# svohr/mixemt

Measured on AMD Instinct MI355X. Metric: read x hap cells/sec through the EM iteration (EM iters/sec reported beside it as em_iters_per_s), 1000000 reads x 5408 haps in total, whole job, higher is better.
Workload: dtype f64

## Files before the change

### mixemt_amd/csrc/coded_kernels.hpp

```cpp
#ifndef MIXEMT_CODED_KERNELS_HPP
#define MIXEMT_CODED_KERNELS_HPP

#define ENC_THREADS 256
#define ENC_SLOTS 1024
#define ENC_MAX_CODES 256
#define ENC_MAX_WIDE 1024
#define ENC_WIDE_SLOTS 4096
#define ENC_EMPTY 0xFFFFFFFFFFFFFFFFull

__host__ __device__ __forceinline__ int rec_code_bytes(int nd, int ldc) { return nd > ENC_MAX_CODES ? 2 * ldc : ldc; }
__device__ __forceinline__ int rec_code_at(const uint8_t *codes, int h, bool wide) {
    return wide ? (int)reinterpret_cast<const uint16_t *>(codes)[h] : (int)codes[h];
}

template <int NCH, bool WIDE>
__device__ __forceinline__ void encode_one_row(int64_t r, const double *__restrict__ M, int64_t ldm, int H, int ldc,
                                               uint8_t *__restrict__ rec, int64_t rec_cap, int64_t *__restrict__ rec_off,
                                               int32_t *__restrict__ ndist, double *__restrict__ rowmax,
                                               unsigned long long *__restrict__ stats) {
    constexpr int NW = ENC_THREADS / 64;
    constexpr int SLOTS = WIDE ? ENC_WIDE_SLOTS : ENC_SLOTS;
    constexpr int MAXC = WIDE ? ENC_MAX_WIDE : ENC_MAX_CODES;
    constexpr int SPT = SLOTS / ENC_THREADS;
    __shared__ unsigned long long s_key[SLOTS];
    __shared__ unsigned short s_code[SLOTS];
    __shared__ double s_red[NW];
    __shared__ int s_wcnt[NW];
    __shared__ int s_flag, s_n;
    __shared__ long long s_off;
    const int t = threadIdx.x, lane = t & 63, wv = t >> 6;
    typedef unsigned int u4 __attribute__((ext_vector_type(4)));
    typedef unsigned int u2 __attribute__((ext_vector_type(2)));

    const auto rsrc = __builtin_amdgcn_make_buffer_rsrc(const_cast<double *>(M + r * ldm), 0, H * 8, 0x00020000);
    double x[NCH][4];
#pragma unroll
    for (int k = 0; k < NCH; ++k) {
        const int off = (t + k * ENC_THREADS) * 32;
        const d2 a = __builtin_bit_cast(d2, (u4)__builtin_amdgcn_raw_buffer_load_b128(rsrc, off, 0, 2));
        const d2 b = __builtin_bit_cast(d2, (u4)__builtin_amdgcn_raw_buffer_load_b128(rsrc, off, 16, 2));
        x[k][0] = a.x;
        x[k][1] = a.y;
        x[k][2] = b.x;
        x[k][3] = b.y;
    }
    if (H & 1) {
        const double tail = M[r * ldm + (H - 1)];
#pragma unroll
        for (int k = 0; k < NCH; ++k) {
            if (4 * (t + k * ENC_THREADS) == H - 1) x[k][0] = tail;
            if (4 * (t + k * ENC_THREADS) + 2 == H - 1) x[k][2] = tail;
        }
    }
#pragma unroll
    for (int q = 0; q < SPT; ++q) s_key[t + q * ENC_THREADS] = ENC_EMPTY;
    if (t == 0) {
        s_flag = 0;
        s_n = 0;
    }
    double m = -INFINITY;
#pragma unroll
    for (int k = 0; k < NCH; ++k)
#pragma unroll
        for (int e = 0; e < 4; ++e)
            if (4 * (t + k * ENC_THREADS) + e < H) m = fmax(m, x[k][e]);
    m = wave_max(m);
    if (lane == 0) s_red[wv] = m;
    __syncthreads();
    m = fmax(fmax(s_red[0], s_red[1]), fmax(s_red[2], s_red[3]));
    const double shift = isfinite(m) ? m : 0.0;

    int slot[NCH][4];
    unsigned long long prev_key = ENC_EMPTY;
    int prev_slot = 0;
#pragma unroll
    for (int k = 0; k < NCH; ++k) {
        const bool give_up = *(volatile int *)&s_flag != 0;
#pragma unroll
        for (int e = 0; e < 4; ++e) {
            const bool valid = 4 * (t + k * ENC_THREADS) + e < H;
            const unsigned long long key = (unsigned long long)__double_as_longlong(x[k][e]);
            int sl = 0;
            bool need = valid;
            if (valid && key == ENC_EMPTY) {
                s_flag = 1;
                need = false;
            }
            if (need && key == prev_key) {
                sl = prev_slot;
                need = false;
            }
            if (give_up) need = false;
            if (need) {
                unsigned int h = (unsigned int)((key ^ (key >> 29)) * 0x9E3779B97F4A7C15ull >> 40) & (SLOTS - 1);
                for (int probes = 0;; ++probes) {
                    const unsigned long long old = atomicCAS(&s_key[h], ENC_EMPTY, key);
                    if (old == ENC_EMPTY) {
                        if (atomicAdd(&s_n, 1) >= MAXC) s_flag = 1;
                        break;
                    }
                    if (old == key) break;
                    h = (h + 1) & (SLOTS - 1);
                    if (probes >= SLOTS) {
                        s_flag = 1;
                        break;
                    }
                }
                sl = (int)h;
            }
            slot[k][e] = sl;
            if (valid) {
                prev_key = key;
                prev_slot = sl;
            }
        }
    }
    __syncthreads();
    const bool dense = (s_flag != 0);

    int cnt = 0;
#pragma unroll
    for (int j = 0; j < SPT; ++j) cnt += (s_key[SPT * t + j] != ENC_EMPTY) ? 1 : 0;
    const int incl = wave_inclusive_scan_i32(cnt);
    if (lane == 63) s_wcnt[wv] = incl;
    __syncthreads();
    int base = 0, D = 0;
#pragma unroll
    for (int q = 0; q < NW; ++q) {
        if (q < wv) base += s_wcnt[q];
        D += s_wcnt[q];
    }
    const int cbytes = WIDE ? 2 * ldc : ldc;
    const int64_t bytes = (int64_t)cbytes + 16 * (int64_t)D;
    const bool coded = !dense && D <= MAXC && (!WIDE || D > ENC_MAX_CODES);
    if (t == 0) {
        long long off = -1;
        if (coded) {
            off = (long long)atomicAdd(&stats[0], (unsigned long long)bytes);
            if (off + bytes > rec_cap) off = -1;
        }
        s_off = off;
    }
    int code = base + incl - cnt;
#pragma unroll
    for (int j = 0; j < SPT; ++j) {
        if (s_key[SPT * t + j] != ENC_EMPTY) s_code[SPT * t + j] = (unsigned short)code++;
    }
    __syncthreads();
    const long long off = s_off;
    if (off >= 0) {
        double *tbl = reinterpret_cast<double *>(rec + off + cbytes);
        code = base + incl - cnt;
#pragma unroll
        for (int j = 0; j < SPT; ++j) {
            const unsigned long long kk = s_key[SPT * t + j];
            if (kk != ENC_EMPTY) {
                const double mval = __longlong_as_double((long long)kk);
                tbl[code] = exp(mval - shift);
                tbl[D + code] = mval;
                ++code;
            }
        }
#pragma unroll
        for (int k = 0; k < NCH; ++k) {
            const int c0 = 4 * (t + k * ENC_THREADS);
            if (c0 < ldc) {
                unsigned int cd[4];
#pragma unroll
                for (int e = 0; e < 4; ++e) cd[e] = (c0 + e < H) ? (unsigned int)s_code[slot[k][e]] : 0u;
                if constexpr (WIDE) {
                    u2 word;
                    word.x = cd[0] | (cd[1] << 16);
                    word.y = cd[2] | (cd[3] << 16);
                    reinterpret_cast<u2 *>(rec + off)[t + k * ENC_THREADS] = word;
                } else {
                    reinterpret_cast<unsigned int *>(rec + off)[t + k * ENC_THREADS] =
                        cd[0] | (cd[1] << 8) | (cd[2] << 16) | (cd[3] << 24);
                }
            }
        }
    }
    if (t == 0) {
        if constexpr (WIDE) {
            if (off >= 0) {
                ndist[r] = D;
                rec_off[r] = off;
                atomicAdd(&stats[1], ~0ull);
            }
        } else {
            rowmax[r] = shift;
            ndist[r] = (off >= 0) ? D : 0;
            rec_off[r] = (off >= 0) ? off : 0;
            if (off < 0) atomicAdd(&stats[1], 1ull);
        }
    }
    __syncthreads();
}

template <int NCH>
__global__ __launch_bounds__(ENC_THREADS) void encode_rows_kernel(
    const double *__restrict__ M, int64_t ldm, int64_t R, int H, int ldc, uint8_t *__restrict__ rec, int64_t rec_cap,
    int64_t *__restrict__ rec_off, int32_t *__restrict__ ndist, double *__restrict__ rowmax,
    unsigned long long *__restrict__ stats) {
    for (int64_t r = blockIdx.x; r < R; r += gridDim.x)
        encode_one_row<NCH, false>(r, M, ldm, H, ldc, rec, rec_cap, rec_off, ndist, rowmax, stats);
}

template <int NCH>
__global__ __launch_bounds__(ENC_THREADS) void encode_wide_rows_kernel(
    const double *__restrict__ M, int64_t ldm, int64_t R, int H, int ldc, uint8_t *__restrict__ rec, int64_t rec_cap,
    int64_t *__restrict__ rec_off, int32_t *__restrict__ ndist, double *__restrict__ rowmax,
    unsigned long long *__restrict__ stats) {
    constexpr int CH = 32;
    __shared__ int s_list[CH];
    __shared__ int s_nlist;
    const int t = threadIdx.x;
    const int64_t nchunk = (R + CH - 1) / CH;
    for (int64_t c = blockIdx.x; c < nchunk; c += gridDim.x) {
        if (t == 0) s_nlist = 0;
        __syncthreads();
        const int64_t r = c * CH + t;
        if (t < CH && r < R && ndist[r] == 0) s_list[atomicAdd(&s_nlist, 1)] = t;
        __syncthreads();
        const int n = s_nlist;
        for (int i = 0; i < n; ++i)
            encode_one_row<NCH, true>(c * CH + s_list[i], M, ldm, H, ldc, rec, rec_cap, rec_off, ndist, rowmax, stats);
        __syncthreads();
    }
}

template <int THREADS, int NCH, int NBUF, bool NT, bool RESIDENT, bool WIDE_PREFETCH, bool CHECK = false>
__device__ __forceinline__ void coded_row_pass(const uint8_t *__restrict__ rec, const int64_t *__restrict__ rec_off,
                                               const int32_t *__restrict__ ndist, int ldc, const double *__restrict__ w,
                                               const int64_t *__restrict__ wide_rows, int64_t n_wide, int64_t R,
                                               const double (&p)[NCH][4], double (&acc)[NCH][4], bool &meta_ready,
                                               int *chk_result = nullptr, const int64_t *__restrict__ row_list = nullptr,
                                               int64_t n_list = 0, const int32_t *__restrict__ nquad = nullptr, int vbid = -1,
                                               int vgrid = 0) {
    static_assert(NBUF >= 3, "codes NBUF - 1 rows ahead, tables NBUF - 2");
    constexpr int NW = THREADS / 64;
    constexpr int AUX = NT ? 2 : 0;
    __shared__ double s_tbl[NBUF][ENC_MAX_CODES];
    __shared__ __attribute__((aligned(16))) double red[NBUF][NW];
    const int t = threadIdx.x, lane = t & 63, wv = t >> 6;
    const int nword = ldc >> 2;
    const int64_t bid = vbid >= 0 ? (int64_t)vbid : (int64_t)blockIdx.x, grid = vbid >= 0 ? (int64_t)vgrid : (int64_t)gridDim.x;
    const row_deal deal(row_list != nullptr ? n_list : R, bid, grid);
    const int voff = t * 4;
    int last_w = t + (NCH - 1) * THREADS;
    if (last_w > nword - 1) last_w = nword - 1;
    const int voff_last = last_w * 4;
    const bool tbl_thread = (THREADS <= ENC_MAX_CODES) || t < ENC_MAX_CODES;
    const int tslot = t & (ENC_MAX_CODES - 1);
    typedef unsigned int u2v __attribute__((ext_vector_type(2)));
    __shared__ int s_chk[2];
    if constexpr (CHECK) {
        if (t == 0) s_chk[0] = s_chk[1] = 0;
        __syncthreads();
    }
    auto list_row = [&](int64_t e) -> int64_t {
        int64_t r = wide_rows[e];
        if constexpr (CHECK) {
            if (r < 0 || r >= R || (e > 0 && wide_rows[e - 1] >= r)) {
                s_chk[1] = 1;
                r = -1;
            }
        }
        return r;
    };
    auto list_nd = [&](int64_t r) -> int {
        if (r < 0) return 0;
        int nd = ndist[r];
        if constexpr (CHECK) {
            if (nd <= ENC_MAX_CODES) {
                s_chk[1] = 1;
                nd = 0;
            }
        }
        return nd;
    };

    __shared__ long long s_off[2][THREADS];
    __shared__ double s_wr[2][THREADS];
    __shared__ int s_nd[2][THREADS];
    auto fetch_meta = [&](int half, int64_t q0) {
        const int64_t q = q0 + t;
        int64_t r = deal.row(q);
        bool struck = false;
        if (row_list != nullptr) {
            const int64_t e = r;
            r = row_list[e];
            if constexpr (CHECK) {
                if (r < 0 || r >= R || (e > 0 && row_list[e - 1] >= r)) {
                    s_chk[1] = 1;
                    r = 0;
                    struck = true;
                }
            }
        }
        int nd = ndist[r];
        if (nd > ENC_MAX_CODES) {
            if constexpr (CHECK) {
                if (row_list != nullptr) s_chk[1] = 1;
                else if (deal.live(q)) atomicAdd(&s_chk[0], 1);
            }
            nd = 0;
        }
        if constexpr (CHECK) {
            if (row_list != nullptr && !struck && (nd <= 0 || nquad[r] != 0)) {
                s_chk[1] = 1;
                struck = true;
            }
        }
        if (struck) nd = 0;
        s_off[half][t] = rec_off[r];
        s_nd[half][t] = nd;
        s_wr[half][t] = (deal.live(q) && nd > 0) ? (w != nullptr ? w[r] : 1.0) : 0.0;
    };

    unsigned int cw[NBUF][NCH];
    double tring[NBUF];
    int pre_off_lo, pre_off_hi, pre_nd;
    double pre_wr;
    auto read_meta = [&](int64_t q_load, int64_t q_weight) {
        const int half = (int)((q_load / THREADS) & 1), idx = (int)(q_load % THREADS);
        const long long off = s_off[half][idx];
        pre_nd = __builtin_amdgcn_readfirstlane(s_nd[half][idx]);
        pre_off_hi = __builtin_amdgcn_readfirstlane((int)(off >> 32));
        pre_off_lo = __builtin_amdgcn_readfirstlane((int)off);
        pre_wr = s_wr[(q_weight / THREADS) & 1][q_weight % THREADS];
    };
    auto load_row = [&](unsigned int(&cws)[NCH], double &tbl_entry) {
        const int nd = pre_nd;
        const uint8_t *base = rec + (((long long)pre_off_hi << 32) | (unsigned int)pre_off_lo);
        const auto rs = __builtin_amdgcn_make_buffer_rsrc(const_cast<uint8_t *>(base), 0, ldc, 0x00020000);
#pragma unroll
        for (int k = 0; k < NCH - 1; ++k) cws[k] = __builtin_amdgcn_raw_buffer_load_b32(rs, voff, k * THREADS * 4, AUX);
        cws[NCH - 1] = __builtin_amdgcn_raw_buffer_load_b32(rs, voff_last, 0, AUX);
        if (tbl_thread) {
            const auto rt = __builtin_amdgcn_make_buffer_rsrc(const_cast<uint8_t *>(base + ldc), 0, nd * 8, 0x00020000);
            const u2v v = __builtin_amdgcn_raw_buffer_load_b64(rt, tslot * 8, 0, AUX);
            tbl_entry = __hiloint2double((int)v.y, (int)v.x);
        }
    };

    const unsigned int three = 3;
    auto entry_off = [&](unsigned int word, auto E) -> unsigned int {
        constexpr int e = decltype(E)::value;
        unsigned int r;
        if constexpr (e == 0) asm("v_lshlrev_b32_sdwa %0, %1, %2 dst_sel:DWORD dst_unused:UNUSED_PAD src0_sel:DWORD src1_sel:BYTE_0" : "=v"(r) : "v"(three), "v"(word));
        else if constexpr (e == 1) asm("v_lshlrev_b32_sdwa %0, %1, %2 dst_sel:DWORD dst_unused:UNUSED_PAD src0_sel:DWORD src1_sel:BYTE_1" : "=v"(r) : "v"(three), "v"(word));
        else if constexpr (e == 2) asm("v_lshlrev_b32_sdwa %0, %1, %2 dst_sel:DWORD dst_unused:UNUSED_PAD src0_sel:DWORD src1_sel:BYTE_2" : "=v"(r) : "v"(three), "v"(word));
        else asm("v_lshlrev_b32_sdwa %0, %1, %2 dst_sel:DWORD dst_unused:UNUSED_PAD src0_sel:DWORD src1_sel:BYTE_3" : "=v"(r) : "v"(three), "v"(word));
        return r;
    };
    auto lookup = [&](const char *tb, unsigned int word, auto E) -> double {
        return *reinterpret_cast<const double *>(tb + entry_off(word, E));
    };
    using E0 = std::integral_constant<int, 0>;
    using E1 = std::integral_constant<int, 1>;
    using E2 = std::integral_constant<int, 2>;
    using E3 = std::integral_constant<int, 3>;

    double v[NCH][4];
    auto lookup_row = [&](const char *tb, const unsigned int(&cws)[NCH]) {
#pragma unroll
        for (int k = 0; k < NCH; ++k) {
            v[k][0] = lookup(tb, cws[k], E0{});
            v[k][1] = lookup(tb, cws[k], E1{});
            v[k][2] = lookup(tb, cws[k], E2{});
            v[k][3] = lookup(tb, cws[k], E3{});
        }
    };

    auto step = [&](auto J, int64_t q) {
        constexpr int j = decltype(J)::value;
        constexpr int jn = (j + 1) % NBUF, jl = (j + NBUF - 1) % NBUF;
        if constexpr (!RESIDENT) {
            if ((q % THREADS) == 0) fetch_meta((int)((q / THREADS + 1) & 1), q + THREADS);
        }
// ... 343 lines not shown
```

### mixemt_amd/csrc/mixemt_hip.hip

```cpp
#include <hip/hip_runtime.h>
#include <stdint.h>
#include <stdio.h>
#include <stdlib.h>
#include <string.h>
#include <math.h>
#include <algorithm>
#include <atomic>
#include <mutex>
#include <type_traits>
#include <utility>
#include <vector>

#include "mixemt_hip.h"
#include "mixemt_hip_tuning.h"

#include "common.hpp"
#include "aln_encode.hpp"
#include "bam_reader.hpp"
#include "coded_kernels.hpp"
#include "quad_kernels.hpp"
#include "quad_batched_kernels.hpp"
#include "build_kernels.hpp"
#include "build_lut_kernels.hpp"
#include "build_sparse_kernels.hpp"
// ... 633 lines not shown
static int em_iter_f32_one(const float *P, int64_t ldp, const double *w, const double *props, int64_t R, int H,
                           const mxm_em_state *state, double *colsum, double *partial, hipStream_t stream,
                           bool timed) {
    const int64_t ldpart = part_ld(H);
    const int nch = ((H + 3) / 4 + MXM_F32_THREADS - 1) / MXM_F32_THREADS;
    const int nbuf = MXM_F32_NBUF;
    int cap = num_cu() * MXM_F32_WG_PER_CU;
    if (cap > MXM_MAX_WG) cap = MXM_MAX_WG;
    const int nwg = clamp_grid((R + nbuf - 1) / nbuf, cap);
    if (timed && T.ev_start != nullptr) HIP_TRY(hipEventRecord(T.ev_start, stream));
    switch (nch) {
#define F32_CASE(n) case n: { const int lrc = launch_wide_f32<n>(P, ldp, w, props, R, H, nwg, partial, ldpart, state, stream); if (lrc != 0) return lrc; } break;
        F32_CASE(1) F32_CASE(2) F32_CASE(3) F32_CASE(4) F32_CASE(5) F32_CASE(6) F32_CASE(7) F32_CASE(8)
#undef F32_CASE
        default: return fail(-1, "mxm_em_iter_f32: H=%s%lld outside the kernel's range", "", H);
    }
    HIP_TRY(hipGetLastError());
    if (timed && T.ev_stop != nullptr) HIP_TRY(hipEventRecord(T.ev_stop, stream));
    hipLaunchKernelGGL(colreduce_kernel, dim3((H + 63) / 64, 1), dim3(COLRED_THREADS), 0, stream, partial, ldpart, nwg,
                       1, H, (const double *)nullptr, colsum, const_cast<mxm_em_state *>(state), slots_from(0), wide_check{nullptr, 0, 0});
    HIP_TRY(hipGetLastError());
    return 0;
}

#define MXM_NARROW_MAX_H 64
template <bool ITER>
static int launch_narrow(const double *M, int64_t ldm, const double *w, const double *ln_props, int64_t R, int H,
                         double *out, int64_t ldo, int mode, double *partial, int64_t ldpart,
                         const mxm_em_state *state, hipStream_t stream, int *nwg_out) {
    const int cap = num_cu() * 4 < MXM_MAX_WG ? num_cu() * 4 : MXM_MAX_WG;
    const int rows_per_wg = (H <= 32) ? 256 : 128;
    const int nwg = clamp_grid((R + rows_per_wg - 1) / rows_per_wg, cap);
    *nwg_out = nwg;
#define NARROW_LAUNCH(hmax, lpr)                                                                             \
    hipLaunchKernelGGL((estep_narrow_kernel<hmax, ITER, lpr>), dim3(nwg), dim3(256), 0, stream, M, ldm, w, ln_props, R, H, \
                       out, ldo, mode, partial, ldpart, state)
    if (H <= 4) NARROW_LAUNCH(4, 1);
    else if (H <= 8) NARROW_LAUNCH(8, 1);
    else if (H <= 16) NARROW_LAUNCH(16, 1);
    else if (H <= 32) NARROW_LAUNCH(32, 1);
    else NARROW_LAUNCH(32, 2);
#undef NARROW_LAUNCH
    HIP_TRY(hipGetLastError());
    return 0;
}

static int em_iter_log_one(const double *M, int64_t ldm, const double *w, const double *ln_props, int64_t R, int H,
                           const mxm_em_state *state, double *colsum, double *partial, hipStream_t stream) {
    if (M == nullptr) return fail(-1, "mxm_em_iter: M is NULL and the linear path does not apply%s", "");
    if (ln_props == nullptr) return fail(-1, "mxm_em_iter: ln_props is NULL and the log-space path needs it%s", "");
    const size_t lds = 2 * (size_t)H * sizeof(double);
    const int64_t ldpart = part_ld(H);
    int nwg;
    if (lds > 150 * 1024) {
        nwg = clamp_grid(R, num_cu() * 2 < MXM_MAX_WG ? num_cu() * 2 : MXM_MAX_WG);
        hipLaunchKernelGGL((estep_global_kernel<true>), dim3(nwg), dim3(ROW_THREADS), 0, stream, M, ldm, w, ln_props, R, H,
                           (double *)nullptr, (int64_t)0, 0, partial, ldpart, state, (const int64_t *)nullptr);
        HIP_TRY(hipGetLastError());
    } else if (H <= MXM_NARROW_MAX_H) {
        const int rc = launch_narrow<true>(M, ldm, w, ln_props, R, H, (double *)nullptr, (int64_t)0, 0, partial, ldpart,
                                           state, stream, &nwg);
        if (rc != 0) return rc;
    } else {
        nwg = clamp_grid(R, num_cu() * 2 < MXM_MAX_WG ? num_cu() * 2 : MXM_MAX_WG);
        if (lds > 60 * 1024 && raise_dynamic_lds(reinterpret_cast<const void *>(&estep_log_kernel<true>), lds, "estep_log_kernel") != hipSuccess)
            return -2;
        hipLaunchKernelGGL((estep_log_kernel<true>), dim3(nwg), dim3(ROW_THREADS), lds, stream, M, ldm, w, ln_props,
                           R, H, (double *)nullptr, (int64_t)0, 0, partial, ldpart, state);
        HIP_TRY(hipGetLastError());
    }
    hipLaunchKernelGGL(colreduce_kernel, dim3((H + 63) / 64, 1), dim3(COLRED_THREADS), 0, stream, partial, ldpart, nwg, 1,
                       H, (const double *)nullptr, colsum, const_cast<mxm_em_state *>(state), slots_from(0), wide_check{nullptr, 0, 0});
    HIP_TRY(hipGetLastError());
    return 0;
}

extern "C" int mxm_em_iter(const double *M, int64_t ldm, const double *P, int64_t ldp, const double *w,
                           const double *props, const double *ln_props, int64_t R, int32_t H, int32_t B,
                           const mxm_em_state *state, double *colsum, void *ws, size_t ws_bytes, void *stream) {
    MXM_ENTER();
    if (R <= 0 || H <= 0 || B <= 0) return fail(-1, "mxm_em_iter: bad shape R=%s%lld H=%lld", "", R, H);
    if (ws == nullptr || ws_bytes < mxm_workspace_bytes(R, H, B)) return fail(-1, "mxm_em_iter: workspace too small%s", "");
    if (P != nullptr && ((ldp & 1) || ldp < H)) return fail(-1, "mxm_em_iter: ldp must be even and >= H%s", "");
    if (M != nullptr && ldm < H) return fail(-1, "mxm_em_iter: ldm < H%s", "");
    const bool linear = (P != nullptr) && mxm_linear_supported(H);
    int max_bt = linear ? T.max_bt : 1;
    while (max_bt > 1 && !batch_fits((int)H, max_bt)) --max_bt;
    for (int b = 0; b < B;) {
        const int left = B - b;
        const int passes = (left + max_bt - 1) / max_bt;
        const int nb = (left + passes - 1) / passes;
        const mxm_em_state *st = state ? state + b : nullptr;
        int rc;
        if (linear)
            rc = em_iter_linear_tile(P, ldp, w, props, R, (int)H, nb, slots_from(b), state, colsum, (double *)ws,
                                     (hipStream_t)stream, b == 0);
        else
            rc = em_iter_log_one(M, ldm, w, ln_props ? ln_props + (int64_t)b * H : nullptr, R, (int)H, st,
                                 colsum + (int64_t)b * H, (double *)ws, (hipStream_t)stream);
        if (rc != 0) return rc;
        b += nb;
    }
    return 0;
}

extern "C" int mxm_linearize_f32(const double *M, int64_t ldm, int64_t R, int32_t H, float *P, int64_t ldp,
                                 double *rowmax, void *stream) {
    if (R < 0 || H <= 0) return fail(-1, "mxm_linearize_f32: bad shape%s", "");
    if (ldm < H || ldp < H || (ldp & 3)) return fail(-1, "mxm_linearize_f32: ldp must be a multiple of 4 and >= H%s (ldp=%lld)", "", ldp);
    if (R == 0) return 0;
    if (wide_rows_ok(M, ldm, H) && (reinterpret_cast<uintptr_t>(P) & 7) == 0 && (ldp & 1) == 0 &&
        linearize_wide<float>(M, ldm, R, (int)H, P, ldp, rowmax, (hipStream_t)stream) == 0) {
        HIP_TRY(hipGetLastError());
        return 0;
    }
    const int grid = clamp_grid(R, num_cu() * 8);
    hipLaunchKernelGGL(linearize_f32_kernel, dim3(grid), dim3(ROW_THREADS), 0, (hipStream_t)stream, M, ldm, R, (int)H,
                       P, ldp, rowmax);
    HIP_TRY(hipGetLastError());
    return 0;
}

extern "C" int mxm_em_iter_f32(const float *P, int64_t ldp, const double *w, const double *props, int64_t R,
                               int32_t H, int32_t B, const mxm_em_state *state, double *colsum, void *ws,
                               size_t ws_bytes, void *stream) {
    MXM_ENTER();
    if (R <= 0 || H <= 0 || B <= 0) return fail(-1, "mxm_em_iter_f32: bad shape R=%s%lld H=%lld", "", R, H);
    if (!mxm_linear_supported(H)) return fail(-1, "mxm_em_iter_f32: H=%s%lld outside the linear kernel's range", "", H);
    if (P == nullptr || (ldp & 3) || ldp < H) return fail(-1, "mxm_em_iter_f32: ldp must be a multiple of 4 and >= H%s", "");
    if (ws == nullptr || ws_bytes < mxm_workspace_bytes(R, H, B)) return fail(-1, "mxm_em_iter_f32: workspace too small%s", "");
    for (int b = 0; b < B; ++b) {
        const int rc = em_iter_f32_one(P, ldp, w, props + (int64_t)b * H, R, (int)H, state ? state + b : nullptr,
                                       colsum + (int64_t)b * H, (double *)ws, (hipStream_t)stream, b == 0);
        if (rc != 0) return rc;
    }
    return 0;
}

extern "C" size_t mxm_coded_bytes(int64_t R, int32_t H) { return mxm_record_bytes(R, H); }

extern "C" int mxm_encode_rows(const double *M, int64_t ldm, int64_t R, int32_t H, uint8_t *rec, size_t rec_bytes,
                               int64_t *rec_off, int32_t *ndist, double *rowmax, int64_t *stats, void *stream) {
    if (R <= 0 || H <= 0 || ldm < H) return fail(-1, "mxm_encode_rows: bad shape R=%s%lld H=%lld", "", R, H);
    if (!mxm_linear_supported(H) || (reinterpret_cast<uintptr_t>(M) & 7) != 0)
        return fail(-1, "mxm_encode_rows: needs H in [65, 8192]%s (H=%lld ldm=%lld)", "", H, ldm);
    if (rec == nullptr || (reinterpret_cast<uintptr_t>(rec) & 15) || rec_bytes < (size_t)coded_ld(H) + 16 * ENC_MAX_CODES)
        return fail(-1, "mxm_encode_rows: record buffer missing, unaligned or smaller than one record%s", "");
    if (rec_off == nullptr || ndist == nullptr || rowmax == nullptr || stats == nullptr)
        return fail(-1, "mxm_encode_rows: output arrays required%s", "");
    hipStream_t s = (hipStream_t)stream;
    HIP_TRY(hipMemsetAsync(stats, 0, 2 * sizeof(int64_t), s));
    const int ldc = coded_ld(H);
    const int nch = (ldc / 4 + ENC_THREADS - 1) / ENC_THREADS;
    const int grid = clamp_grid(R, num_cu() * 4);
    const int grid_w = clamp_grid((R + 31) / 32, num_cu() * 3);
    switch (nch) {
#define ENC_CASE(n) case n: hipLaunchKernelGGL((encode_rows_kernel<n>), dim3(grid), dim3(ENC_THREADS), 0, s, M, ldm, R, (int)H, ldc, rec, (int64_t)rec_bytes, rec_off, ndist, rowmax, reinterpret_cast<unsigned long long *>(stats)); \
                    hipLaunchKernelGGL((encode_wide_rows_kernel<n>), dim3(grid_w), dim3(ENC_THREADS), 0, s, M, ldm, R, (int)H, ldc, rec, (int64_t)rec_bytes, rec_off, ndist, rowmax, reinterpret_cast<unsigned long long *>(stats)); break;
        ENC_CASE(1) ENC_CASE(2) ENC_CASE(3) ENC_CASE(4) ENC_CASE(5) ENC_CASE(6) ENC_CASE(7) ENC_CASE(8)
#undef ENC_CASE
        default: return fail(-1, "mxm_encode_rows: H=%s%lld outside the kernel's range", "", H);
    }
    HIP_TRY(hipGetLastError());
    return 0;
}

static int coded_check(const mxm_coded *c, int32_t H, const char *who) {
    if (c == nullptr || c->R <= 0 || H <= 0 || !mxm_linear_supported(H))
        return fail(-1, "%s: bad coded matrix (rows %lld, H %lld)", who, c ? c->R : 0, H);
    if (c->rec == nullptr || c->rec_off == nullptr || c->ndist == nullptr) return fail(-1, "%s: coded matrix arrays missing", who);
    if (c->R_rest < 0 || (c->R_rest > 0 && (c->P_rest == nullptr || c->ldp_rest < H || (c->ldp_rest & 1) ||
                                            (reinterpret_cast<uintptr_t>(c->P_rest) & 15))))
        return fail(-1, "%s: the dense rest needs 16-byte aligned rows with an even ld >= H", who);
    if (c->n_wide < 0 || (c->n_wide > 0 && c->wide_rows == nullptr)) return fail(-1, "%s: n_wide > 0 needs wide_rows", who);
    if (c->qrec != nullptr) {
        if (c->qoff == nullptr || c->nquad == nullptr || c->n_quad_rows < 0 || c->n_byte_rows < 0 ||
            (c->n_quad_rows > 0 && c->quad_rows == nullptr) || (c->n_byte_rows > 0 && c->byte_rows == nullptr) ||
            (reinterpret_cast<uintptr_t>(c->qrec) & 31))
            return fail(-1, "%s: quad dictionary arrays missing (or qrec not 32-byte aligned)", who);
        if (c->n_quad_rows + c->n_byte_rows + c->n_wide + c->R_rest != c->R)
            return fail(-1, "%s: quad_rows + byte_rows + wide_rows + the dense rest must be all %lld rows", who, c->R);
    }
    return 0;
}

extern "C" size_t mxm_quad_bytes(int64_t R, int32_t H) {
    (void)H;
    constexpr size_t largest = QUAD_CODE_BYTES + QUAD_MAX * 32, per_piece = (size_t)QUAD_CHUNK / largest;
    return R > 0 ? (((size_t)R + per_piece - 1) / per_piece + 5120) * (size_t)QUAD_CHUNK : 0;
}

extern "C" int mxm_expand_tables(const uint8_t *maj, const int32_t *mk_ptr, const uint16_t *mk_hap, const uint8_t *mk_base,
                                 const uint8_t *map256, int32_t S, int32_t H, int64_t lde, uint8_t *out, void *stream) {
    if (maj == nullptr || mk_ptr == nullptr || mk_hap == nullptr || mk_base == nullptr || out == nullptr || S <= 0 || H <= 0 || lde < H)
        return fail(-1, "mxm_expand_tables: bad arguments%s", "");
    hipLaunchKernelGGL(expand_tables_kernel, dim3(clamp_grid(S, num_cu() * 8)), dim3(256), 0, (hipStream_t)stream, maj, mk_ptr, mk_hap,
                       mk_base, map256, (int)S, (int)H, lde, out);
    HIP_TRY(hipGetLastError());
    return 0;
}

extern "C" size_t mxm_quad_lists_scratch_bytes(int64_t R) {
    return R > 0 ? (size_t)((R + QLIST_CHUNK - 1) / QLIST_CHUNK) * 2 * sizeof(long long) : 0;
}

extern "C" int mxm_quad_lists(const int32_t *ndist, const int32_t *nquad, int64_t R, int64_t *quad_rows, int64_t *byte_rows,
                              int64_t *counts, void *scratch, size_t scratch_bytes, void *stream) {
    MXM_ENTER();
    if (ndist == nullptr || nquad == nullptr || R <= 0 || quad_rows == nullptr || byte_rows == nullptr || counts == nullptr)
        return fail(-1, "mxm_quad_lists: bad arguments%s", "");
    if (scratch == nullptr || scratch_bytes < mxm_quad_lists_scratch_bytes(R)) return fail(-1, "mxm_quad_lists: scratch too small%s", "");
    const int64_t nchunk = (R + QLIST_CHUNK - 1) / QLIST_CHUNK;
    if (nchunk > 0x7fffffff) return fail(-1, "mxm_quad_lists: too many rows%s", "");
    hipStream_t s = (hipStream_t)stream;
    long long *cc = static_cast<long long *>(scratch);
    hipLaunchKernelGGL(quad_list_count_kernel, dim3((unsigned)nchunk), dim3(QLIST_THREADS), 0, s, ndist, nquad, R, cc);
    hipLaunchKernelGGL(quad_list_scan_kernel, dim3(1), dim3(QLIST_THREADS), 0, s, cc, nchunk, reinterpret_cast<long long *>(counts));
    hipLaunchKernelGGL(quad_list_fill_kernel, dim3((unsigned)nchunk), dim3(QLIST_THREADS), 0, s, ndist, nquad, R, cc, quad_rows, byte_rows);
    HIP_TRY(hipGetLastError());
    return 0;
}

extern "C" int mxm_build_quads(const mxm_coded *c, int32_t H, uint8_t *qrec, size_t qrec_bytes, int64_t *qoff, int32_t *nquad,
                               uint64_t *stats, void *stream) {
    MXM_ENTER();
    if (c == nullptr || c->R <= 0 || c->rec == nullptr || c->rec_off == nullptr || c->ndist == nullptr || !mxm_linear_supported(H))
        return fail(-1, "mxm_build_quads: bad coded matrix (rows %s%lld, H %lld)", "", c ? c->R : 0, H);
    if (qoff == nullptr || nquad == nullptr || stats == nullptr || (qrec == nullptr && qrec_bytes > 0) ||
        (reinterpret_cast<uintptr_t>(qrec) & 31))
        return fail(-1, "mxm_build_quads: qoff, nquad, stats and a 32-byte aligned qrec required%s", "");
    const int ldc = coded_ld(H);
    if (ldc / 4 > 8 * QUAD_THREADS) return fail(-1, "mxm_build_quads: H=%s%lld beyond eight quads per thread", "", H);
    HIP_TRY(hipMemsetAsync(stats, 0, 2 * sizeof(uint64_t), (hipStream_t)stream));
    if (T.quad_encoder == 1 && ldc / 4 <= 64 * QW_K)
        hipLaunchKernelGGL(quad_encode_wave_kernel, dim3(clamp_grid((c->R + QW_WAVES - 1) / QW_WAVES, std::min(num_cu() * QW_MIN_WAVES, 5120 / QW_WAVES))), dim3(QUAD_THREADS),
                           0, (hipStream_t)stream, c->rec, c->rec_off, c->ndist, ldc, (int)H, c->R, qrec,
                           (unsigned long long)qrec_bytes, qoff, nquad, reinterpret_cast<unsigned long long *>(stats));
    else
        hipLaunchKernelGGL(quad_encode_kernel, dim3(clamp_grid(c->R, num_cu() * 8)), dim3(QUAD_THREADS), 0, (hipStream_t)stream,
                           c->rec, c->rec_off, c->ndist, ldc, (int)H, c->R, qrec, (unsigned long long)qrec_bytes, qoff, nquad,
                           reinterpret_cast<unsigned long long *>(stats));
    HIP_TRY(hipGetLastError());
    return 0;
}

extern "C" int mxm_decode_rows(const mxm_coded *c, int32_t H, double *P, int64_t ldp, void *stream) {
    const int rc = coded_check(c, H, "mxm_decode_rows");
    if (rc != 0) return rc;
    if (P == nullptr || ldp < H) return fail(-1, "mxm_decode_rows: ldp < H%s", "");
    hipLaunchKernelGGL(decode_rows_kernel, dim3(clamp_grid(c->R, num_cu() * 8)), dim3(256), 0, (hipStream_t)stream, c->rec,
                       c->rec_off, c->ndist, coded_ld(H), c->R, (int)H, P, ldp);
    HIP_TRY(hipGetLastError());
    return 0;
}

extern "C" int mxm_row_argmax_votes_coded(const mxm_coded *c, int32_t H, int32_t n_runs, const double *ln_props,
                                          const double *props, const double *rowmax, const double *M_rest, int64_t ldm_rest,
                                          const int64_t *rest_rows, int64_t n_rest, const double *w, int32_t *best,
                                          double *votes, void *ws, size_t ws_bytes, void *stream) {
    const int rc = coded_check(c, H, "mxm_row_argmax_votes_coded");
    if (rc != 0) return rc;
    if (ln_props == nullptr || best == nullptr || n_runs < 1 || n_runs > RECK_MAX_RUNS)
        return fail(-1, "mxm_row_argmax_votes_coded: ln_props, best and 1..%s%lld runs required", "", (long long)RECK_MAX_RUNS);
    if (n_runs > 1 && (props == nullptr || rowmax == nullptr))
        return fail(-1, "mxm_row_argmax_votes_coded: several runs need props and rowmax (each run's row normaliser)%s", "");
    if (n_rest < 0 || (n_rest > 0 && (M_rest == nullptr || rest_rows == nullptr || ldm_rest < H)))
        return fail(-1, "mxm_row_argmax_votes_coded: the rows without a record need M_rest, rest_rows and ldm_rest >= H%s", "");
    if (votes != nullptr && (ws == nullptr || ws_bytes < mxm_workspace_bytes(c->R, H, 1)))
        return fail(-1, "mxm_row_argmax_votes_coded: workspace too small%s", "");
    hipStream_t s = (hipStream_t)stream;
    const size_t lse_lds = (size_t)n_runs * sizeof(double);
    const int ldc_a = coded_ld(H);
    const int nch_a = (ldc_a / 4 + 255) / 256;
    bool fast = n_runs == 1 && nch_a <= 8;
    if (fast) {
        switch (nch_a) {
#define RA_CASE(n) case n: { int per_cu = 2; if (hipOccupancyMaxActiveBlocksPerMultiprocessor(&per_cu, records_argmax_narrow_kernel<n>, 256, 0) != hipSuccess || per_cu < 1) { (void)hipGetLastError(); per_cu = 2; } \
                hipLaunchKernelGGL((records_argmax_narrow_kernel<n>), dim3(clamp_grid(c->R, num_cu() * per_cu)), dim3(256), 0, s, c->rec, c->rec_off, c->ndist, ldc_a, c->R, (int)H, ln_props, best); \
                 \
                hipLaunchKernelGGL((records_argmax_kernel<n, true>), dim3(clamp_grid((c->R + 255) / 256, num_cu() * 2)), dim3(256), 0, s, c->rec, c->rec_off, c->ndist, ldc_a, c->R, (int)H, ln_props, best, (const int64_t *)nullptr); } break;
            RA_CASE(1) RA_CASE(2) RA_CASE(3) RA_CASE(4) RA_CASE(5) RA_CASE(6) RA_CASE(7) RA_CASE(8)
#undef RA_CASE
            default: fast = false;
        }
    }
    if (!fast)
        hipLaunchKernelGGL(posterior_argmax_kernel<true>, dim3(clamp_grid(c->R, num_cu() * 8)), dim3(256), lse_lds, s, c->rec, c->rec_off,
                           c->ndist, coded_ld(H), (const double *)nullptr, (int64_t)0, (const int64_t *)nullptr, c->R, (int)H,
                           (int)n_runs, ln_props, props, rowmax, best);
    HIP_TRY(hipGetLastError());
    if (n_rest > 0) {
        hipLaunchKernelGGL(posterior_argmax_kernel<false>, dim3(clamp_grid(n_rest, num_cu() * 8)), dim3(256), lse_lds, s,
                           (const uint8_t *)nullptr, (const int64_t *)nullptr, (const int32_t *)nullptr, 0, M_rest, ldm_rest,
                           rest_rows, n_rest, (int)H, (int)n_runs, ln_props, props, rowmax, best);
        HIP_TRY(hipGetLastError());
    }
    if (votes != nullptr) {
        const int64_t ldpart = part_ld(H);
        const int nwg = clamp_grid((c->R + 255) / 256, num_cu() * 2 < MXM_MAX_WG ? num_cu() * 2 : MXM_MAX_WG);
        const size_t vlds = (size_t)H * sizeof(double);
        if (vlds > 150 * 1024) return fail(-1, "mxm_row_argmax_votes_coded: H=%s%lld too wide for the vote kernel", "", H);
        if (vlds > 60 * 1024 && raise_dynamic_lds(reinterpret_cast<const void *>(&votes_from_best_kernel), vlds, "votes_from_best_kernel") != hipSuccess)
            return -2;
        hipLaunchKernelGGL(votes_from_best_kernel, dim3(nwg), dim3(256), vlds, s, best, w, c->R, (int)H, (double *)ws, ldpart);
        HIP_TRY(hipGetLastError());
        hipLaunchKernelGGL(colreduce_kernel, dim3((H + 63) / 64, 1), dim3(COLRED_THREADS), 0, s, (const double *)ws, ldpart, nwg,
                           1, (int)H, (const double *)nullptr, votes, (mxm_em_state *)nullptr, slots_from(0), wide_check{nullptr, 0, 0});
        HIP_TRY(hipGetLastError());
    }
    return 0;
}
// ... 1387 lines not shown
```

Measured before the change: 879.4 billion.

## Fuse narrow and wide row encoding into one pass with prefetched rows

The two encode kernels (a narrow pass, then a wide-code pass re-reading rows that failed) are merged into a single kernel. It uses a 4096-slot hash table, assigns codes at insertion time through an inverse slot map instead of a block scan, and chooses byte or 16-bit codes per row. It also double-buffers row loads so the next row is prefetched while the current one is encoded. The table is cleared incrementally rather than fully per row. This removes a second pass over the matrix and a scan, but code order now depends on atomic insertion order, and the larger shared memory lowers occupancy.

New measurement: 881.6 billion, median of 2. About the same (+0.2%).

```diff
diff --git a/mixemt_amd/csrc/coded_kernels.hpp b/mixemt_amd/csrc/coded_kernels.hpp
--- a/mixemt_amd/csrc/coded_kernels.hpp
+++ b/mixemt_amd/csrc/coded_kernels.hpp
@@ -2,10 +2,9 @@
 #define MIXEMT_CODED_KERNELS_HPP
 
 #define ENC_THREADS 256
-#define ENC_SLOTS 1024
 #define ENC_MAX_CODES 256
 #define ENC_MAX_WIDE 1024
-#define ENC_WIDE_SLOTS 4096
+#define ENC_SLOTS 4096
 #define ENC_EMPTY 0xFFFFFFFFFFFFFFFFull
 
 __host__ __device__ __forceinline__ int rec_code_bytes(int nd, int ldc) { return nd > ENC_MAX_CODES ? 2 * ldc : ldc; }
@@ -13,219 +12,201 @@
     return wide ? (int)reinterpret_cast<const uint16_t *>(codes)[h] : (int)codes[h];
 }
 
-template <int NCH, bool WIDE>
-__device__ __forceinline__ void encode_one_row(int64_t r, const double *__restrict__ M, int64_t ldm, int H, int ldc,
-                                               uint8_t *__restrict__ rec, int64_t rec_cap, int64_t *__restrict__ rec_off,
-                                               int32_t *__restrict__ ndist, double *__restrict__ rowmax,
-                                               unsigned long long *__restrict__ stats) {
+template <int NCH>
+__global__ __launch_bounds__(ENC_THREADS, 2) void encode_rows_kernel(
+    const double *__restrict__ M, int64_t ldm, int64_t R, int H, int ldc, uint8_t *__restrict__ rec, int64_t rec_cap,
+    int64_t *__restrict__ rec_off, int32_t *__restrict__ ndist, double *__restrict__ rowmax,
+    unsigned long long *__restrict__ stats) {
     constexpr int NW = ENC_THREADS / 64;
-    constexpr int SLOTS = WIDE ? ENC_WIDE_SLOTS : ENC_SLOTS;
-    constexpr int MAXC = WIDE ? ENC_MAX_WIDE : ENC_MAX_CODES;
-    constexpr int SPT = SLOTS / ENC_THREADS;
-    __shared__ unsigned long long s_key[SLOTS];
-    __shared__ unsigned short s_code[SLOTS];
+    constexpr int SPT = ENC_SLOTS / ENC_THREADS;
+    __shared__ unsigned long long s_key[ENC_SLOTS];
+    __shared__ unsigned short s_code[ENC_SLOTS];
+    __shared__ unsigned short s_inv[ENC_MAX_WIDE];
     __shared__ double s_red[NW];
-    __shared__ int s_wcnt[NW];
     __shared__ int s_flag, s_n;
     __shared__ long long s_off;
     const int t = threadIdx.x, lane = t & 63, wv = t >> 6;
     typedef unsigned int u4 __attribute__((ext_vector_type(4)));
     typedef unsigned int u2 __attribute__((ext_vector_type(2)));
-
-    const auto rsrc = __builtin_amdgcn_make_buffer_rsrc(const_cast<double *>(M + r * ldm), 0, H * 8, 0x00020000);
-    double x[NCH][4];
-#pragma unroll
-    for (int k = 0; k < NCH; ++k) {
-        const int off = (t + k * ENC_THREADS) * 32;
-        const d2 a = __builtin_bit_cast(d2, (u4)__builtin_amdgcn_raw_buffer_load_b128(rsrc, off, 0, 2));
-        const d2 b = __builtin_bit_cast(d2, (u4)__builtin_amdgcn_raw_buffer_load_b128(rsrc, off, 16, 2));
-        x[k][0] = a.x;
-        x[k][1] = a.y;
-        x[k][2] = b.x;
-        x[k][3] = b.y;
-    }
-    if (H & 1) {
-        const double tail = M[r * ldm + (H - 1)];
+    const row_deal deal(R);
+    const bool odd = (H & 1) != 0;
+
+    auto load_row = [&](int64_t q, double(&x)[NCH][4], double &tail) {
+        const auto rsrc = __builtin_amdgcn_make_buffer_rsrc(const_cast<double *>(M + deal.row(q) * ldm), 0,
+                                                            deal.live(q) ? H * 8 : 0, 0x00020000);
 #pragma unroll
         for (int k = 0; k < NCH; ++k) {
-            if (4 * (t + k * ENC_THREADS) == H - 1) x[k][0] = tail;
-            if (4 * (t + k * ENC_THREADS) + 2 == H - 1) x[k][2] = tail;
-        }
-    }
-#pragma unroll
-    for (int q = 0; q < SPT; ++q) s_key[t + q * ENC_THREADS] = ENC_EMPTY;
-    if (t == 0) {
-        s_flag = 0;
-        s_n = 0;
-    }
-    double m = -INFINITY;
-#pragma unroll
-    for (int k = 0; k < NCH; ++k)
-#pragma unroll
-        for (int e = 0; e < 4; ++e)
-            if (4 * (t + k * ENC_THREADS) + e < H) m = fmax(m, x[k][e]);
-    m = wave_max(m);
-    if (lane == 0) s_red[wv] = m;
-    __syncthreads();
-    m = fmax(fmax(s_red[0], s_red[1]), fmax(s_red[2], s_red[3]));
-    const double shift = isfinite(m) ? m : 0.0;
-
-    int slot[NCH][4];
-    unsigned long long prev_key = ENC_EMPTY;
-    int prev_slot = 0;
-#pragma unroll
-    for (int k = 0; k < NCH; ++k) {
-        const bool give_up = *(volatile int *)&s_flag != 0;
-#pragma unroll
-        for (int e = 0; e < 4; ++e) {
-            const bool valid = 4 * (t + k * ENC_THREADS) + e < H;
-            const unsigned long long key = (unsigned long long)__double_as_longlong(x[k][e]);
-            int sl = 0;
-            bool need = valid;
-            if (valid && key == ENC_EMPTY) {
-                s_flag = 1;
-                need = false;
-            }
-            if (need && key == prev_key) {
-                sl = prev_slot;
-                need = false;
-            }
-            if (give_up) need = false;
-            if (need) {
-                unsigned int h = (unsigned int)((key ^ (key >> 29)) * 0x9E3779B97F4A7C15ull >> 40) & (SLOTS - 1);
-                for (int probes = 0;; ++probes) {
-                    const unsigned long long old = atomicCAS(&s_key[h], ENC_EMPTY, key);
-                    if (old == ENC_EMPTY) {
-                        if (atomicAdd(&s_n, 1) >= MAXC) s_flag = 1;
-                        break;
+            const int off = (t + k * ENC_THREADS) * 32;
+            const d2 a = __builtin_bit_cast(d2, (u4)__builtin_amdgcn_raw_buffer_load_b128(rsrc, off, 0, 2));
+            const d2 b = __builtin_bit_cast(d2, (u4)__builtin_amdgcn_raw_buffer_load_b128(rsrc, off, 16, 2));
+            x[k][0] = a.x;
+            x[k][1] = a.y;
+            x[k][2] = b.x;
+            x[k][3] = b.y;
+        }
+        if (odd) tail = __builtin_bit_cast(double, (u2)__builtin_amdgcn_raw_buffer_load_b64(rsrc, (H - 1) * 8, 0, 2));
+    };
+
+    auto encode = [&](int64_t q, double(&x)[NCH][4], double &tail, double(&xn)[NCH][4], double &tailn) {
+        const int64_t r = deal.row(q);
+        load_row(q + 1, xn, tailn);
+        if (odd) {
+#pragma unroll
+            for (int k = 0; k < NCH; ++k) {
+                if (4 * (t + k * ENC_THREADS) == H - 1) x[k][0] = tail;
+                if (4 * (t + k * ENC_THREADS) + 2 == H - 1) x[k][2] = tail;
+            }
+        }
+        double m = -INFINITY;
+#pragma unroll
+        for (int k = 0; k < NCH; ++k)
+#pragma unroll
+            for (int e = 0; e < 4; ++e)
+                if (4 * (t + k * ENC_THREADS) + e < H) m = fmax(m, x[k][e]);
+        m = wave_max(m);
+        if (lane == 0) s_red[wv] = m;
+        __syncthreads();
+        m = fmax(fmax(s_red[0], s_red[1]), fmax(s_red[2], s_red[3]));
+        const double shift = isfinite(m) ? m : 0.0;
+
+        int slot[NCH][4];
+        unsigned long long prev_key = ENC_EMPTY;
+        int prev_slot = 0;
+#pragma unroll
+        for (int k = 0; k < NCH; ++k) {
+            const bool give_up = *(volatile int *)&s_flag != 0;
+#pragma unroll
+            for (int e = 0; e < 4; ++e) {
+                const bool valid = 4 * (t + k * ENC_THREADS) + e < H;
+                const unsigned long long key = (unsigned long long)__double_as_longlong(x[k][e]);
+                int sl = 0;
+                bool need = valid;
+                if (valid && key == ENC_EMPTY) {
+                    s_flag = 1;
+                    need = false;
+                }
+                if (need && key == prev_key) {
+                    sl = prev_slot;
+                    need = false;
+                }
+                if (give_up) need = false;
+                if (need) {
+                    unsigned int h = (unsigned int)((key ^ (key >> 29)) * 0x9E3779B97F4A7C15ull >> 40) & (ENC_SLOTS - 1);
+                    for (int probes = 0;; ++probes) {
+                        const unsigned long long old = atomicCAS(&s_key[h], ENC_EMPTY, key);
+                        if (old == ENC_EMPTY) {
+                            const int c = atomicAdd(&s_n, 1);
+                            if (c >= ENC_MAX_WIDE) s_flag = 1;
+                            else {
+                                s_code[h] = (unsigned short)c;
+                                s_inv[c] = (unsigned short)h;
+                            }
+                            break;
+                        }
+                        if (old == key) break;
+                        h = (h + 1) & (ENC_SLOTS - 1);
+                        if (probes >= ENC_SLOTS) {
+                            s_flag = 1;
+                            break;
+                        }
                     }
-                    if (old == key) break;
-                    h = (h + 1) & (SLOTS - 1);
-                    if (probes >= SLOTS) {
-                        s_flag = 1;
-                        break;
+                    sl = (int)h;
+                }
+                slot[k][e] = sl;
+                if (valid) {
+                    prev_key = key;
+                    prev_slot = sl;
+                }
+            }
+        }
+        __syncthreads();
+        const bool dense = (s_flag != 0);
+        const int D = dense ? 0 : s_n;
+        const bool wide = D > ENC_MAX_CODES;
+        const int cbytes = wide ? 2 * ldc : ldc;
+        const int64_t bytes = (int64_t)cbytes + 16 * (int64_t)D;
+        if (t == 0) {
+            long long off = -1;
+            if (!dense) {
+                off = (long long)atomicAdd(&stats[0], (unsigned long long)bytes);
+                if (off + bytes > rec_cap) off = -1;
+            }
+            s_off = off;
+        }
+        if (!dense) {
+#pragma unroll
+            for (int k = 0; k < NCH; ++k)
+#pragma unroll
+                for (int e = 0; e < 4; ++e)
+                    slot[k][e] = (4 * (t + k * ENC_THREADS) + e < H) ? (int)s_code[slot[k][e]] : 0;
+        } else {
+#pragma unroll
+            for (int j = 0; j < SPT; ++j) s_key[t + j * ENC_THREADS] = ENC_EMPTY;
+        }
+        double mval0 = 0.0, pval0 = 0.0;
+        if (t < D) {
+            const int h = s_inv[t];
+            mval0 = __longlong_as_double((long long)s_key[h]);
+            s_key[h] = ENC_EMPTY;
+            pval0 = exp(mval0 - shift);
+        }
+        __syncthreads();
+        const long long off = s_off;
+        double *tbl = reinterpret_cast<double *>(rec + off + cbytes);
+        if (t < D && off >= 0) {
+            tbl[t] = pval0;
+            tbl[D + t] = mval0;
+        }
+        for (int c = t + ENC_THREADS; c < D; c += ENC_THREADS) {
+            const int h = s_inv[c];
+            const double mval = __longlong_as_double((long long)s_key[h]);
+            s_key[h] = ENC_EMPTY;
+            if (off >= 0) {
+                tbl[c] = exp(mval - shift);
+                tbl[D + c] = mval;
+            }
+        }
+        if (off >= 0) {
+#pragma unroll
+            for (int k = 0; k < NCH; ++k) {
+                const int c0 = 4 * (t + k * ENC_THREADS);
+                if (c0 < ldc) {
+                    const unsigned int c0v = (unsigned int)slot[k][0], c1v = (unsigned int)slot[k][1],
+                                       c2v = (unsigned int)slot[k][2], c3v = (unsigned int)slot[k][3];
+                    if (wide) {
+                        u2 word;
+                        word.x = c0v | (c1v << 16);
+                        word.y = c2v | (c3v << 16);
+                        reinterpret_cast<u2 *>(rec + off)[t + k * ENC_THREADS] = word;
+                    } else {
+                        reinterpret_cast<unsigned int *>(rec + off)[t + k * ENC_THREADS] =
+                            c0v | (c1v << 8) | (c2v << 16) | (c3v << 24);
                     }
                 }
-                sl = (int)h;
-            }
-            slot[k][e] = sl;
-            if (valid) {
-                prev_key = key;
-                prev_slot = sl;
-            }
-        }
-    }
-    __syncthreads();
-    const bool dense = (s_flag != 0);
-
-    int cnt = 0;
-#pragma unroll
-    for (int j = 0; j < SPT; ++j) cnt += (s_key[SPT * t + j] != ENC_EMPTY) ? 1 : 0;
-    const int incl = wave_inclusive_scan_i32(cnt);
-    if (lane == 63) s_wcnt[wv] = incl;
-    __syncthreads();
-    int base = 0, D = 0;
-#pragma unroll
-    for (int q = 0; q < NW; ++q) {
-        if (q < wv) base += s_wcnt[q];
-        D += s_wcnt[q];
-    }
-    const int cbytes = WIDE ? 2 * ldc : ldc;
-    const int64_t bytes = (int64_t)cbytes + 16 * (int64_t)D;
-    const bool coded = !dense && D <= MAXC && (!WIDE || D > ENC_MAX_CODES);
-    if (t == 0) {
-        long long off = -1;
-        if (coded) {
-            off = (long long)atomicAdd(&stats[0], (unsigned long long)bytes);
-            if (off + bytes > rec_cap) off = -1;
-        }
-        s_off = off;
-    }
-    int code = base + incl - cnt;
-#pragma unroll
-    for (int j = 0; j < SPT; ++j) {
-        if (s_key[SPT * t + j] != ENC_EMPTY) s_code[SPT * t + j] = (unsigned short)code++;
-    }
-    __syncthreads();
-    const long long off = s_off;
-    if (off >= 0) {
-        double *tbl = reinterpret_cast<double *>(rec + off + cbytes);
-        code = base + incl - cnt;
-#pragma unroll
-        for (int j = 0; j < SPT; ++j) {
-            const unsigned long long kk = s_key[SPT * t + j];
-            if (kk != ENC_EMPTY) {
-                const double mval = __longlong_as_double((long long)kk);
-                tbl[code] = exp(mval - shift);
-                tbl[D + code] = mval;
-                ++code;
-            }
-        }
-#pragma unroll
-        for (int k = 0; k < NCH; ++k) {
-            const int c0 = 4 * (t + k * ENC_THREADS);
-            if (c0 < ldc) {
-                unsigned int cd[4];
-#pragma unroll
-                for (int e = 0; e < 4; ++e) cd[e] = (c0 + e < H) ? (unsigned int)s_code[slot[k][e]] : 0u;
-                if constexpr (WIDE) {
-                    u2 word;
-                    word.x = cd[0] | (cd[1] << 16);
-                    word.y = cd[2] | (cd[3] << 16);
-                    reinterpret_cast<u2 *>(rec + off)[t + k * ENC_THREADS] = word;
-                } else {
-                    reinterpret_cast<unsigned int *>(rec + off)[t + k * ENC_THREADS] =
-                        cd[0] | (cd[1] << 8) | (cd[2] << 16) | (cd[3] << 24);
-                }
-            }
-        }
-    }
-    if (t == 0) {
-        if constexpr (WIDE) {
-            if (off >= 0) {
-                ndist[r] = D;
-                rec_off[r] = off;
-                atomicAdd(&stats[1], ~0ull);
-            }
-        } else {
+            }
+        }
+        if (t == 0) {
             rowmax[r] = shift;
             ndist[r] = (off >= 0) ? D : 0;
             rec_off[r] = (off >= 0) ? off : 0;
             if (off < 0) atomicAdd(&stats[1], 1ull);
-        }
-    }
-    __syncthreads();
-}
-
-template <int NCH>
-__global__ __launch_bounds__(ENC_THREADS) void encode_rows_kernel(
-    const double *__restrict__ M, int64_t ldm, int64_t R, int H, int ldc, uint8_t *__restrict__ rec, int64_t rec_cap,
-    int64_t *__restrict__ rec_off, int32_t *__restrict__ ndist, double *__restrict__ rowmax,
-    unsigned long long *__restrict__ stats) {
-    for (int64_t r = blockIdx.x; r < R; r += gridDim.x)
-        encode_one_row<NCH, false>(r, M, ldm, H, ldc, rec, rec_cap, rec_off, ndist, rowmax, stats);
-}
-
-template <int NCH>
-__global__ __launch_bounds__(ENC_THREADS) void encode_wide_rows_kernel(
-    const double *__restrict__ M, int64_t ldm, int64_t R, int H, int ldc, uint8_t *__restrict__ rec, int64_t rec_cap,
-    int64_t *__restrict__ rec_off, int32_t *__restrict__ ndist, double *__restrict__ rowmax,
-    unsigned long long *__restrict__ stats) {
-    constexpr int CH = 32;
-    __shared__ int s_list[CH];
-    __shared__ int s_nlist;
-    const int t = threadIdx.x;
-    const int64_t nchunk = (R + CH - 1) / CH;
-    for (int64_t c = blockIdx.x; c < nchunk; c += gridDim.x) {
-        if (t == 0) s_nlist = 0;
-        __syncthreads();
-        const int64_t r = c * CH + t;
-        if (t < CH && r < R && ndist[r] == 0) s_list[atomicAdd(&s_nlist, 1)] = t;
-        __syncthreads();
-        const int n = s_nlist;
-        for (int i = 0; i < n; ++i)
-            encode_one_row<NCH, true>(c * CH + s_list[i], M, ldm, H, ldc, rec, rec_cap, rec_off, ndist, rowmax, stats);
-        __syncthreads();
+            s_flag = 0;
+            s_n = 0;
+        }
+    };
+
+#pragma unroll
+    for (int j = 0; j < SPT; ++j) s_key[t + j * ENC_THREADS] = ENC_EMPTY;
+    if (t == 0) {
+        s_flag = 0;
+        s_n = 0;
+    }
+    double xa[NCH][4], xb[NCH][4], ta = 0.0, tb = 0.0;
+    load_row(0, xa, ta);
+    for (int64_t q = 0; q < deal.nq; q += 2) {
+        encode(q, xa, ta, xb, tb);
+        if (q + 1 >= deal.nq) break;
+        encode(q + 1, xb, tb, xa, ta);
     }
 }
 
diff --git a/mixemt_amd/csrc/mixemt_hip.hip b/mixemt_amd/csrc/mixemt_hip.hip
--- a/mixemt_amd/csrc/mixemt_hip.hip
+++ b/mixemt_amd/csrc/mixemt_hip.hip
@@ -809,11 +809,9 @@
     HIP_TRY(hipMemsetAsync(stats, 0, 2 * sizeof(int64_t), s));
     const int ldc = coded_ld(H);
     const int nch = (ldc / 4 + ENC_THREADS - 1) / ENC_THREADS;
-    const int grid = clamp_grid(R, num_cu() * 4);
-    const int grid_w = clamp_grid((R + 31) / 32, num_cu() * 3);
+    const int grid = clamp_grid(R, num_cu() * 2);
     switch (nch) {
-#define ENC_CASE(n) case n: hipLaunchKernelGGL((encode_rows_kernel<n>), dim3(grid), dim3(ENC_THREADS), 0, s, M, ldm, R, (int)H, ldc, rec, (int64_t)rec_bytes, rec_off, ndist, rowmax, reinterpret_cast<unsigned long long *>(stats)); \
-                    hipLaunchKernelGGL((encode_wide_rows_kernel<n>), dim3(grid_w), dim3(ENC_THREADS), 0, s, M, ldm, R, (int)H, ldc, rec, (int64_t)rec_bytes, rec_off, ndist, rowmax, reinterpret_cast<unsigned long long *>(stats)); break;
+#define ENC_CASE(n) case n: hipLaunchKernelGGL((encode_rows_kernel<n>), dim3(grid), dim3(ENC_THREADS), 0, s, M, ldm, R, (int)H, ldc, rec, (int64_t)rec_bytes, rec_off, ndist, rowmax, reinterpret_cast<unsigned long long *>(stats)); break;
         ENC_CASE(1) ENC_CASE(2) ENC_CASE(3) ENC_CASE(4) ENC_CASE(5) ENC_CASE(6) ENC_CASE(7) ENC_CASE(8)
 #undef ENC_CASE
         default: return fail(-1, "mxm_encode_rows: H=%s%lld outside the kernel's range", "", H);
```
